# DIG-Beihang/RobustART

Hardware: AMD Instinct MI355X
Metric: corrupted+attacked images/sec/node (ResNet-50, PGD-7 + IN-C x5) (higher is better)
Workload: dtype bf16x3; 1 GPU; per step and GPU: gaussian_noise sev 1..5 on 256 u8 224x224 images -> normalise -> ResNet-50 eval (1280 img) + PGD-Linf-7 eps 2/255 ResNet-50 eval (256 img); global_batch=256, parallelism=dp1, streams=2

## Files before the change

### robustart_amd/csrc/stem_pair.hip

```cpp
#include "rart_common.h"

typedef __attribute__((ext_vector_type(8))) __bf16 bf16x8;
typedef __attribute__((ext_vector_type(4))) float f32x4;

namespace {
constexpr int T = 16;
constexpr int HT = T + 3;
constexpr int NPOS_PAD = 368;
constexpr int PT = T / 2 + 3;
constexpr int NPOOL = PT * PT;
constexpr int OT = 2 * T;
constexpr int OLD = OT + 1;
constexpr int DZ_BYTES = 2 * 4 * NPOS_PAD * 16;
constexpr int DP_BYTES = 2 * NPOOL * 4 * 16;
constexpr int ARG_BYTES = NPOOL * 4 * 8;
static_assert(3 * OT * OLD * 4 <= DP_BYTES + ARG_BYTES, "output tile must fit the raw pooled tile");

__device__ __forceinline__ uint32_t sp_pack2(float lo, float hi) {
  typedef __attribute__((ext_vector_type(2))) float f2;
  typedef __attribute__((ext_vector_type(2))) __bf16 b2;
  f2 f = {lo, hi};
  return __builtin_bit_cast(uint32_t, __builtin_convertvector(f, b2));
}

template <int EY, int EX>
__device__ __forceinline__ void pool_bwd_class_pair(uint4* sDz1, const uint4* sDp, const uint2* sArg, int tid, int a0, int b0, int qy0,
                                                    int qx0, int oh, int ow) {
  constexpr int NY = EY ? (HT + 1) / 2 : HT / 2, NX = EX ? (HT + 1) / 2 : HT / 2;
  constexpr int NYS = EY ? 2 : 1, NXS = EX ? 2 : 1;
  for (int i = tid; i < 4 * NY * NX; i += 256) {
    const int c = i / (NY * NX), j = i - c * (NY * NX);
    const int iy = j / NX, ix = j - iy * NX;
    const int hy = 2 * iy + (EY ? 0 : 1), hx = 2 * ix + (EX ? 0 : 1);
    const int py = a0 - 1 + hy, px = b0 - 1 + hx;
    float g[8] = {0.f, 0.f, 0.f, 0.f, 0.f, 0.f, 0.f, 0.f};
    if ((unsigned)py < (unsigned)oh && (unsigned)px < (unsigned)ow) {
#pragma unroll
      for (int ia = 0; ia < NYS; ++ia) {
        const int qy = (py >> 1) + ia;
        const uint32_t ky = (uint32_t)(py - (2 * qy - 1));
#pragma unroll
        for (int ib = 0; ib < NXS; ++ib) {
          const int qx = (px >> 1) + ib;
          const uint32_t mine = (ky * 3 + (uint32_t)(px - (2 * qx - 1))) * 0x01010101u;
          const int lp = (qy - qy0) * PT + (qx - qx0);
          const uint2 cd = sArg[c * NPOOL + lp];
          const uint4 dh = sDp[c * NPOOL + lp], dl = sDp[(4 + c) * NPOOL + lp];
          const uint32_t cw[2] = {cd.x, cd.y};
          const uint32_t hw_[4] = {dh.x, dh.y, dh.z, dh.w}, lw_[4] = {dl.x, dl.y, dl.z, dl.w};
#pragma unroll
          for (int hw = 0; hw < 2; ++hw) {
            const uint32_t ne = ((cw[hw] ^ mine) + 0x7F7F7F7Fu) & 0x80808080u;
            const uint32_t eq = (ne ^ 0x80808080u) >> 7;
            const uint32_t m = (eq << 8) - eq;
            const uint32_t m0 = __builtin_amdgcn_perm(m, m, 0x01010000u), m1 = __builtin_amdgcn_perm(m, m, 0x03030202u);
            const uint32_t h0 = hw_[2 * hw] & m0, h1 = hw_[2 * hw + 1] & m1, l0 = lw_[2 * hw] & m0, l1 = lw_[2 * hw + 1] & m1;
            g[4 * hw + 0] += __uint_as_float(h0 << 16) + __uint_as_float(l0 << 16);
            g[4 * hw + 1] += __uint_as_float(h0 & 0xFFFF0000u) + __uint_as_float(l0 & 0xFFFF0000u);
            g[4 * hw + 2] += __uint_as_float(h1 << 16) + __uint_as_float(l1 << 16);
            g[4 * hw + 3] += __uint_as_float(h1 & 0xFFFF0000u) + __uint_as_float(l1 & 0xFFFF0000u);
          }
        }
      }
    }
    uint32_t hv[4], lv[4];
#pragma unroll
    for (int k = 0; k < 4; ++k) {
      hv[k] = sp_pack2(g[2 * k], g[2 * k + 1]);
      lv[k] = sp_pack2(g[2 * k] - __uint_as_float(hv[k] << 16), g[2 * k + 1] - __uint_as_float(hv[k] & 0xFFFF0000u));
    }
    sDz1[c * NPOS_PAD + hy * HT + hx] = make_uint4(hv[0], hv[1], hv[2], hv[3]);
    sDz1[(4 + c) * NPOS_PAD + hy * HT + hx] = make_uint4(lv[0], lv[1], lv[2], lv[3]);
  }
}

struct Istd3p { float v[3]; };

__global__ __launch_bounds__(256, 2) void k_stem_bwd_pair(const uint4* __restrict__ dpool_h,
                                                          const uint4* __restrict__ dpool_l,
                                                          const uint4* __restrict__ arg,
                                                          const uint16_t* __restrict__ wt_h,
                                                          const uint16_t* __restrict__ wt_l,
                                                          float* __restrict__ grad,
                                                          int h, int w, Istd3p istd) {
  __shared__ __attribute__((aligned(16))) uint8_t lds[DZ_BYTES + DP_BYTES + ARG_BYTES];
  uint4* sDz1 = reinterpret_cast<uint4*>(lds);
  uint4* sDp = reinterpret_cast<uint4*>(lds + DZ_BYTES);
  uint2* sArg = reinterpret_cast<uint2*>(lds + DZ_BYTES + DP_BYTES);
  float* sOut = reinterpret_cast<float*>(lds + DZ_BYTES);

  const int tid = threadIdx.x, lane = tid & 63, wave = tid >> 6;
  const int oh = h >> 1, ow = w >> 1;
  const int oh2 = oh >> 1, ow2 = ow >> 1;
  const int a0 = blockIdx.y * T, b0 = blockIdx.x * T, img = blockIdx.z;
  const int qy0 = (a0 >> 1) - 1, qx0 = (b0 >> 1) - 1;
  const int fr = lane & 15, fg = lane >> 4;
  f32x4 acc[4];
#pragma unroll
  for (int m = 0; m < 4; ++m) acc[m] = (f32x4){0.f, 0.f, 0.f, 0.f};
  const uint4* wrow_h = reinterpret_cast<const uint4*>(wt_h + (size_t)fr * 1024 + fg * 8);
  const uint4* wrow_l = reinterpret_cast<const uint4*>(wt_l + (size_t)fr * 1024 + fg * 8);

#pragma unroll 1
  for (int half = 0; half < 2; ++half) {
    for (int i = tid; i < NPOOL * 10; i += 256) {
      const int pos = i / 10, v = i - pos * 10;
      const int qy = qy0 + pos / PT, qx = qx0 + pos % PT;
      const bool ok = (unsigned)qy < (unsigned)oh2 && (unsigned)qx < (unsigned)ow2;
      const size_t base = ((size_t)img * oh2 + qy) * ow2 + qx;
      if (v < 8) {
        const int pl = v >> 2, c = v & 3;
        uint4 val = make_uint4(0, 0, 0, 0);
        if (ok) val = (pl ? dpool_l : dpool_h)[base * 8 + half * 4 + c];
        sDp[(pl * 4 + c) * NPOOL + pos] = val;
      } else {
        uint4 val = make_uint4(0x0F0F0F0Fu, 0x0F0F0F0Fu, 0x0F0F0F0Fu, 0x0F0F0F0Fu);
        if (ok) val = arg[base * 4 + half * 2 + (v - 8)];
        sArg[(2 * (v - 8)) * NPOOL + pos] = make_uint2(val.x, val.y);
        sArg[(2 * (v - 8) + 1) * NPOOL + pos] = make_uint2(val.z, val.w);
      }
    }
    __syncthreads();
    pool_bwd_class_pair<0, 0>(sDz1, sDp, sArg, tid, a0, b0, qy0, qx0, oh, ow);
    pool_bwd_class_pair<0, 1>(sDz1, sDp, sArg, tid, a0, b0, qy0, qx0, oh, ow);
    pool_bwd_class_pair<1, 0>(sDz1, sDp, sArg, tid, a0, b0, qy0, qx0, oh, ow);
    pool_bwd_class_pair<1, 1>(sDz1, sDp, sArg, tid, a0, b0, qy0, qx0, oh, ow);
    __syncthreads();
#pragma unroll
    for (int dpi = 0; dpi < 4; ++dpi) {
      uint4 bh[4], bl[4];
#pragma unroll
      for (int t = 0; t < 4; ++t) {
        bh[t] = wrow_h[(dpi * 4 + t) * 8 + half * 4];
        bl[t] = wrow_l[(dpi * 4 + t) * 8 + half * 4];
      }
#pragma unroll
      for (int dqi = 0; dqi < 4; ++dqi) {
        const bf16x8 wh = __builtin_bit_cast(bf16x8, bh[dqi]), wl = __builtin_bit_cast(bf16x8, bl[dqi]);
#pragma unroll
        for (int m = 0; m < 4; ++m) {
          const int pos = (wave * 4 + m + dpi) * HT + fr + dqi;
          const bf16x8 ah = __builtin_bit_cast(bf16x8, sDz1[fg * NPOS_PAD + pos]);
          const bf16x8 al = __builtin_bit_cast(bf16x8, sDz1[(4 + fg) * NPOS_PAD + pos]);
          acc[m] = __builtin_amdgcn_mfma_f32_16x16x32_bf16(al, wh, acc[m], 0, 0, 0);
          acc[m] = __builtin_amdgcn_mfma_f32_16x16x32_bf16(ah, wl, acc[m], 0, 0, 0);
          acc[m] = __builtin_amdgcn_mfma_f32_16x16x32_bf16(ah, wh, acc[m], 0, 0, 0);
        }
      }
    }
  }

  if (fr < 12) {
    const int pq = fr / 3, c = fr - pq * 3;
    const int py = pq >> 1, px = pq & 1;
#pragma unroll
    for (int m = 0; m < 4; ++m)
#pragma unroll
      for (int j = 0; j < 4; ++j)
        sOut[(c * OT + 2 * (wave * 4 + m) + py) * OLD + 2 * (fg * 4 + j) + px] = acc[m][j];
  }
  __syncthreads();
  const size_t plane = (size_t)h * w;
  for (int i = tid; i < 3 * OT * (OT / 4); i += 256) {
    const int x4 = i & 7, row = i >> 3;
    const int c = row / OT, y = row - c * OT;
    const int gy = 2 * a0 + y, gx = 2 * b0 + x4 * 4;
    if (gy < h && gx < w) {
      const float s = istd.v[c];
      const float* r = sOut + (c * OT + y) * OLD + x4 * 4;
      *reinterpret_cast<float4*>(grad + ((size_t)img * 3 + c) * plane + (size_t)gy * w + gx) =
          make_float4(r[0] * s, r[1] * s, r[2] * s, r[3] * s);
    }
  }
}
}

extern "C" int rart_engine_stem_bwd_fused_pair(const void* dpool_hi, const void* dpool_lo, const void* argmax, const void* wtab_hi,
                                               const void* wtab_lo, float* grad, int n, int h, int w, const float* std_host,
                                               rart_stream_t stream) {
  RART_CHECK_ARG(dpool_hi && dpool_lo && argmax && wtab_hi && wtab_lo && grad && n > 0 && n <= 65535,
                 "rart_engine_stem_bwd_fused_pair: bad arguments");
  RART_CHECK_ARG(h % 4 == 0 && w % 4 == 0 && h >= 4 && w >= 4, "rart_engine_stem_bwd_fused_pair: h and w must be multiples of 4");
  Istd3p is;
  for (int c = 0; c < 3; ++c) is.v[c] = std_host ? 1.0f / std_host[c] : 1.0f;
  const int oh = h / 2, ow = w / 2;
  hipLaunchKernelGGL(k_stem_bwd_pair, dim3((ow + T - 1) / T, (oh + T - 1) / T, n), dim3(256), 0, (hipStream_t)stream,
                     (const uint4*)dpool_hi, (const uint4*)dpool_lo, (const uint4*)argmax, (const uint16_t*)wtab_hi,
                     (const uint16_t*)wtab_lo, grad, h, w, is);
  RART_CHECK_LAUNCH("rart_engine_stem_bwd_fused_pair");
  return RART_OK;
}

namespace {
typedef __attribute__((ext_vector_type(16))) float f32x16;
constexpr int SP_PT = 8;
constexpr int SP_R = 2 * SP_PT + 1;
constexpr int SP_NPOS = SP_R * SP_R;
constexpr int SP_PH = 2 * (SP_R - 1) + 7;
constexpr int SP_PW = 40;
constexpr int SP_PLANE = SP_PH * SP_PW * 8;
constexpr int SP_WROW = 464;
constexpr int SP_YROW = 272;
constexpr int SP_W_BYTES = 64 * SP_WROW;
constexpr int SP_T_BYTES = SP_NPOS * SP_YROW;
constexpr int SP_NT = 3;
static_assert(SP_T_BYTES >= 2 * SP_PLANE, "the stem-output tile must cover the patch it aliases");

struct StemNormP { float mean[3], istd[3]; };
#pragma clang fp contract(off)

template <bool SRC_U8>
__global__ __launch_bounds__(512, 1) void k_stem_fwd_pair(const void* __restrict__ src, const uint16_t* __restrict__ w_h,
                                                          const uint16_t* __restrict__ w_l, const float* __restrict__ bias,
                                                          uint4* __restrict__ p1_h, uint4* __restrict__ p1_l, uint2* __restrict__ arg,
                                                          uint8_t* __restrict__ sign, int n, int h, int w, StemNormP nm) {
  __shared__ __attribute__((aligned(16))) uint8_t lds[2 * SP_W_BYTES + SP_T_BYTES];
  uint8_t* sW = lds;
  uint8_t* sP = lds + 2 * SP_W_BYTES;
  const int tid = threadIdx.x, lane = tid & 63, wave = tid >> 6;
  const int wm = wave >> 1, wn = wave & 1;
  const int kq = lane >> 5;
  const int oh = h >> 1, ow = w >> 1, oh2 = oh >> 1, ow2 = ow >> 1;
  const int tiles_x = (ow2 + SP_PT - 1) / SP_PT, tiles_y = (oh2 + SP_PT - 1) / SP_PT;
  const int n_tiles = n * tiles_y * tiles_x;

  for (int i = tid; i < 2 * 64 * 28; i += 512) {
    const int pl = i / (64 * 28), j = i - pl * (64 * 28), row = j / 28, ch = j - row * 28;
    *reinterpret_cast<uint4*>(sW + pl * SP_W_BYTES + row * SP_WROW + ch * 16) =
        *reinterpret_cast<const uint4*>((pl ? w_l : w_h) + (size_t)row * 224 + ch * 8);
  }
  uint32_t a_off[SP_NT];
#pragma unroll
  for (int i = 0; i < SP_NT; ++i) {
    int p = (wm * SP_NT + i) * 32 + (lane & 31);
    p = p < SP_NPOS ? p : SP_NPOS - 1;
    const int py = p / SP_R, px = p - py * SP_R;
    a_off[i] = (uint32_t)(((2 * py) * SP_PW + 2 * px) * 8 + kq * 16);
  }
  const uint32_t w_off = (uint32_t)((wn * 32 + (lane & 31)) * SP_WROW + kq * 16);
  float bz[16];
#pragma unroll
  for (int r = 0; r < 16; ++r) bz[r] = bias ? bias[wn * 32 + (r & 3) + 8 * (r >> 2) + 4 * kq] : 0.f;

  for (int t = blockIdx.x; t < n_tiles; t += gridDim.x) {
    const int img = t / (tiles_y * tiles_x);
    const int tr = t - img * (tiles_y * tiles_x);
    const int q0y = (tr / tiles_x) * SP_PT, q0x = (tr % tiles_x) * SP_PT;
    const int in_y0 = 4 * q0y - 5, in_x0 = 4 * q0x - 5;
    __syncthreads();
    {
      constexpr int U = (SP_PH * SP_PW + 511) / 512;
      float v01[U][3];
      bool ok[U];
#pragma unroll
      for (int u = 0; u < U; ++u) {
        const int i = u * 512 + tid;
        const int pr = i / SP_PW, pc = i - pr * SP_PW;
        const int y = in_y0 + pr, x = in_x0 + pc;
        ok[u] = i < SP_PH * SP_PW && (unsigned)y < (unsigned)h && (unsigned)x < (unsigned)w && pc < SP_PH;
#pragma unroll
        for (int c = 0; c < 3; ++c) {
          v01[u][c] = 0.f;
          if (ok[u]) {
            if (SRC_U8) v01[u][c] = (float)((const uint8_t*)src)[(((size_t)img * h + y) * w + x) * 3 + c];
            else v01[u][c] = ((const float*)src)[(((size_t)img * 3 + c) * h + y) * w + x];
          }
        }
      }
#pragma unroll
      for (int u = 0; u < U; ++u) {
        const int i = u * 512 + tid;
        if (i >= SP_PH * SP_PW) continue;
        uint32_t hv[3] = {0, 0, 0}, lv[3] = {0, 0, 0};
        if (ok[u]) {
#pragma unroll
          for (int c = 0; c < 3; ++c) {
            const float x01 = SRC_U8 ? v01[u][c] * (1.0f / 255.0f) : v01[u][c];
            const float v = (x01 - nm.mean[c]) * nm.istd[c];
            hv[c] = sp_pack2(v, 0.f) & 0xFFFFu;
            lv[c] = sp_pack2(v - __uint_as_float(hv[c] << 16), 0.f) & 0xFFFFu;
          }
        }
        *reinterpret_cast<uint2*>(sP + i * 8) = make_uint2(hv[0] | (hv[1] << 16), hv[2]);
        *reinterpret_cast<uint2*>(sP + SP_PLANE + i * 8) = make_uint2(lv[0] | (lv[1] << 16), lv[2]);
      }
    }
    __syncthreads();
    f32x16 acc[SP_NT];
#pragma unroll
    for (int i = 0; i < SP_NT; ++i)
#pragma unroll
      for (int r = 0; r < 16; ++r) acc[i][r] = bz[r];
#pragma unroll
    for (int r = 0; r < 7; ++r)
#pragma unroll
      for (int ks = 0; ks < 2; ++ks) {
        const bf16x8 wh = *reinterpret_cast<const bf16x8*>(sW + w_off + r * 64 + ks * 32);
        const bf16x8 wl = *reinterpret_cast<const bf16x8*>(sW + SP_W_BYTES + w_off + r * 64 + ks * 32);
#pragma unroll
        for (int i = 0; i < SP_NT; ++i) {
          const bf16x8 ah = *reinterpret_cast<const bf16x8*>(sP + a_off[i] + r * (SP_PW * 8) + ks * 32);
          const bf16x8 al = *reinterpret_cast<const bf16x8*>(sP + a_off[i] + SP_PLANE + r * (SP_PW * 8) + ks * 32);
          acc[i] = __builtin_amdgcn_mfma_f32_32x32x16_bf16(wh, al, acc[i], 0, 0, 0);
          acc[i] = __builtin_amdgcn_mfma_f32_32x32x16_bf16(wl, ah, acc[i], 0, 0, 0);
          acc[i] = __builtin_amdgcn_mfma_f32_32x32x16_bf16(wh, ah, acc[i], 0, 0, 0);
        }
      }
    __syncthreads();
#pragma unroll
    for (int i = 0; i < SP_NT; ++i) {
      const int p = (wm * SP_NT + i) * 32 + (lane & 31);
      if (p < SP_NPOS) {
#pragma unroll
        for (int q = 0; q < 4; ++q) {
          float v[4];
#pragma unroll
          for (int k = 0; k < 4; ++k) v[k] = fmaxf(acc[i][4 * q + k], 0.f);
          const uint32_t h0 = sp_pack2(v[0], v[1]), h1 = sp_pack2(v[2], v[3]);
          const uint32_t l0 = sp_pack2(v[0] - __uint_as_float(h0 << 16), v[1] - __uint_as_float(h0 & 0xFFFF0000u));
          const uint32_t l1 = sp_pack2(v[2] - __uint_as_float(h1 << 16), v[3] - __uint_as_float(h1 & 0xFFFF0000u));
          *reinterpret_cast<float4*>(sP + p * SP_YROW + (wn * 32 + 8 * q + 4 * kq) * 4) =
              make_float4(__uint_as_float(h0 << 16) + __uint_as_float(l0 << 16), __uint_as_float(h0 & 0xFFFF0000u) + __uint_as_float(l0 & 0xFFFF0000u),
                          __uint_as_float(h1 << 16) + __uint_as_float(l1 << 16), __uint_as_float(h1 & 0xFFFF0000u) + __uint_as_float(l1 & 0xFFFF0000u));
        }
      }
    }
    __syncthreads();
    {
      const int c = tid & 7, q = tid >> 3;
      const int qy = q / SP_PT, qx = q - qy * SP_PT;
      const int gy = q0y + qy, gx = q0x + qx;
      if (gy < oh2 && gx < ow2) {
        float m[8];
        uint32_t code[8];
#pragma unroll
        for (int j = 0; j < 8; ++j) { m[j] = -INFINITY; code[j] = 0; }
        for (int ky = 0; ky < 3; ++ky) {
          const int y1 = 2 * gy - 1 + ky;
          if ((unsigned)y1 >= (unsigned)oh) continue;
          for (int kx = 0; kx < 3; ++kx) {
            const int x1 = 2 * gx - 1 + kx;
            if ((unsigned)x1 >= (unsigned)ow) continue;
            const float* tp = reinterpret_cast<const float*>(sP + ((2 * qy + ky) * SP_R + 2 * qx + kx) * SP_YROW) + c * 8;
            const float4 v0 = *reinterpret_cast<const float4*>(tp), v1 = *reinterpret_cast<const float4*>(tp + 4);
            const float f[8] = {v0.x, v0.y, v0.z, v0.w, v1.x, v1.y, v1.z, v1.w};
#pragma unroll
            for (int j = 0; j < 8; ++j)
              if (f[j] > m[j]) { m[j] = f[j]; code[j] = (uint32_t)(ky * 3 + kx); }
          }
        }
        const size_t o = (((size_t)img * oh2 + gy) * ow2 + gx) * 8 + c;
        uint32_t hv[4], lv[4];
#pragma unroll
        for (int k = 0; k < 4; ++k) {
          hv[k] = sp_pack2(m[2 * k], m[2 * k + 1]);
          lv[k] = sp_pack2(m[2 * k] - __uint_as_float(hv[k] << 16), m[2 * k + 1] - __uint_as_float(hv[k] & 0xFFFF0000u));
        }
        p1_h[o] = make_uint4(hv[0], hv[1], hv[2], hv[3]);
        p1_l[o] = make_uint4(lv[0], lv[1], lv[2], lv[3]);
        uint32_t sb = 0;
#pragma unroll
        for (int j = 0; j < 8; ++j) {
          if (m[j] > 0.f) sb |= 1u << j; else code[j] = 15u;
        }
        if (sign) sign[o] = (uint8_t)sb;
        if (arg) arg[o] = make_uint2(code[0] | (code[1] << 8) | (code[2] << 16) | (code[3] << 24),
                                     code[4] | (code[5] << 8) | (code[6] << 16) | (code[7] << 24));
      }
    }
  }
}
#pragma clang fp contract(fast)
}

extern "C" int rart_engine_stem_fwd_fused_pair(const void* src, int src_is_u8, const void* wgt_hi, const void* wgt_lo, const float* bias,
                                               void* p1_hi, void* p1_lo, void* argmax_out, void* sign_out, int n, int h, int w,
                                               const float* mean_host, const float* std_host, rart_stream_t stream) {
  RART_CHECK_ARG(src && wgt_hi && wgt_lo && p1_hi && p1_lo && n > 0 && h % 4 == 0 && w % 4 == 0 && h >= 4 && w >= 4,
                 "rart_engine_stem_fwd_fused_pair: bad arguments (h, w multiples of 4)");
  StemNormP nm;
  for (int c = 0; c < 3; ++c) {
    nm.mean[c] = mean_host ? mean_host[c] : 0.f;
    nm.istd[c] = std_host ? 1.0f / std_host[c] : 1.f;
  }
  const long long tiles = (long long)n * ((h / 4 + SP_PT - 1) / SP_PT) * ((w / 4 + SP_PT - 1) / SP_PT);
  const int grid = (int)(tiles < 256 ? tiles : 256);
  if (src_is_u8)
    hipLaunchKernelGGL(k_stem_fwd_pair<true>, dim3(grid), dim3(512), 0, (hipStream_t)stream, src, (const uint16_t*)wgt_hi,
                       (const uint16_t*)wgt_lo, bias, (uint4*)p1_hi, (uint4*)p1_lo, (uint2*)argmax_out, (uint8_t*)sign_out, n, h, w, nm);
  else
    hipLaunchKernelGGL(k_stem_fwd_pair<false>, dim3(grid), dim3(512), 0, (hipStream_t)stream, src, (const uint16_t*)wgt_hi,
                       (const uint16_t*)wgt_lo, bias, (uint4*)p1_hi, (uint4*)p1_lo, (uint2*)argmax_out, (uint8_t*)sign_out, n, h, w, nm);
  RART_CHECK_LAUNCH("rart_engine_stem_fwd_fused_pair");
  return RART_OK;
}
```

Measured before the change: 8228 images/s.

## Restructure stem kernels: prefetch next tiles, stage weights in LDS, pad layouts

In the stem backward kernel, the raw pooled-gradient and argmax tile for the next half is now loaded into registers while the current half is being computed. The MFMA weights are staged into LDS, in a region that aliases the raw tile, instead of being reloaded from global memory per pass. Pooled data moves to a padded, channel-interleaved layout to reduce LDS bank conflicts. The forward kernel prefetches the next tile's input patch (f32 path by default, u8 opt-in), pads the patch row stride, and rebalances m-tiles across waves. Optional timestamp instrumentation and profiling scripts are also added. The cost is more registers, more barriers, and a risk of lower occupancy.

```diff
diff --git a/profiles/stem_pair_ab.py b/profiles/stem_pair_ab.py
--- /dev/null
+++ b/profiles/stem_pair_ab.py
@@ -0,0 +1,73 @@
+import ctypes, json, os, subprocess, sys
+ROOT = os.path.dirname(os.path.dirname(os.path.abspath(__file__)))
+sys.path.insert(0, ROOT)
+
+if sys.argv[1] == '--kernels-child':
+    from robustart_amd import _lib
+    _lib.LIB_PATH = os.path.abspath(sys.argv[2])
+    import torch
+    from robustart_amd.model.engine import ResNet50Engine
+    from robustart_amd.model.engine_base import pair
+    lib = _lib.load()
+    B, H, W = 256, 224, 224
+    g = torch.Generator().manual_seed(5)
+    wb = torch.randn(64, 3, 7, 7, generator=g) * 0.1
+    wt = pair(ResNet50Engine._stem_bwd_table(wb, dtype=torch.float32)).cuda()
+    rows = torch.zeros(64, 7, 8, 4); rows[:, :, :7, :3] = wb.permute(0, 2, 3, 1)
+    wf = pair(rows.reshape(64, 224)).cuda()
+    bias = torch.randn(64, generator=g).cuda()
+    xf = torch.rand(B, 3, H, W, generator=g).cuda()
+    xu = torch.randint(0, 256, (B, H, W, 3), generator=g, dtype=torch.uint8).cuda()
+    p1 = torch.empty(2, B, H // 4, W // 4, 64, dtype=torch.bfloat16, device='cuda')
+    arg = torch.empty(B, H // 4, W // 4, 64, dtype=torch.uint8, device='cuda')
+    sign = torch.empty(B, H // 4, W // 4, 8, dtype=torch.uint8, device='cuda')
+    dp = pair(torch.randn(B, H // 4, W // 4, 64, generator=g)).cuda()
+    grad = torch.empty(B, 3, H, W, device='cuda')
+    m3 = (ctypes.c_float * 3)(0.485, 0.456, 0.406); s3 = (ctypes.c_float * 3)(0.229, 0.224, 0.225)
+    sp = _lib.stream_ptr()
+    fwd = lambda x, u8: _lib.check(lib.rart_engine_stem_fwd_fused_pair(_lib.ptr(x), u8, _lib.ptr(wf[0]), _lib.ptr(wf[1]), _lib.ptr(bias), _lib.ptr(p1[0]), _lib.ptr(p1[1]), _lib.ptr(arg), _lib.ptr(sign), B, H, W, m3, s3, sp))
+    bwd = lambda: _lib.check(lib.rart_engine_stem_bwd_fused_pair(_lib.ptr(dp[0]), _lib.ptr(dp[1]), _lib.ptr(arg), _lib.ptr(wt[0]), _lib.ptr(wt[1]), _lib.ptr(grad), B, H, W, s3, sp))
+    def t(fn, n=30):
+        for _ in range(5): fn()
+        torch.cuda.synchronize()
+        e0, e1 = torch.cuda.Event(enable_timing=True), torch.cuda.Event(enable_timing=True)
+        e0.record()
+        for _ in range(n): fn()
+        e1.record(); torch.cuda.synchronize()
+        return round(e0.elapsed_time(e1) / n * 1e3, 1)
+    print(json.dumps({'lib': sys.argv[2], 'fwd_f32_us': t(lambda: fwd(xf, 0)), 'fwd_u8_us': t(lambda: fwd(xu, 1)), 'bwd_us': t(bwd)}), flush=True)
+    sys.exit(0)
+if sys.argv[1] == '--bench-child':
+    import runpy
+    from robustart_amd import _lib
+    _lib.LIB_PATH = os.path.abspath(sys.argv[2])
+    sys.argv = [os.path.join(ROOT, 'bench.py')] + sys.argv[3:]
+    runpy.run_path(sys.argv[0], run_name='__main__')
+    sys.exit(0)
+
+mode, args = sys.argv[1], sys.argv[2:]
+rounds = int(args[args.index('--rounds') + 1]) if '--rounds' in args else (2 if mode == 'kernels' else 4)
+dump = args[args.index('--dump') + 1] if '--dump' in args else None
+libs = [a for a in args if a.endswith('.so')]
+for r in range(rounds):
+    for n, lib in enumerate(libs):
+        if mode == 'kernels':
+            cmd = [sys.executable, os.path.abspath(__file__), '--kernels-child', lib]
+        else:
+            cmd = [sys.executable, os.path.abspath(__file__), '--bench-child', lib, '--gpus', '1', '--steps', '20', '--warmup', '5']
+            if dump and r == 0:
+                cmd += ['--dump-outputs', os.path.join(dump, str(n))]
+        o = subprocess.run(cmd, capture_output=True, text=True, timeout=600)
+        line = [ln for ln in o.stdout.splitlines() if ln.startswith('{')]
+        if o.returncode != 0 or not line:
+            sys.exit('child failed for %s:\n%s' % (lib, o.stderr[-2000:]))
+        j = json.loads(line[-1])
+        print(json.dumps(j if mode == 'kernels' else {'lib': lib, 'round': r, 'ms_per_step': j['ms_per_step'], 'value': j['value']}), flush=True)
+if mode == 'bench' and dump:
+    import numpy as np
+    a, b = os.path.join(dump, '0'), os.path.join(dump, '1')
+    names = sorted(os.listdir(a))
+    assert names and names == sorted(os.listdir(b))
+    bad = [n for n in names if not np.array_equal(np.load(os.path.join(a, n)), np.load(os.path.join(b, n)))]
+    print(json.dumps({'dump_outputs_arrays': len(names), 'array_equal': not bad, 'different': bad}), flush=True)
+    sys.exit(1 if bad else 0)
diff --git a/profiles/stem_pair_lab_build.py b/profiles/stem_pair_lab_build.py
--- /dev/null
+++ b/profiles/stem_pair_lab_build.py
@@ -0,0 +1,23 @@
+import os
+import subprocess
+import sys
+
+ROOT = os.path.dirname(os.path.dirname(os.path.abspath(__file__)))
+sys.path.insert(0, ROOT)
+from robustart_amd.csrc import build as B
+
+
+def main(argv):
+    out, defs, src = argv[0], [a for a in argv[1:] if a.startswith('-D')], os.path.join(B.HERE, 'stem_pair.hip')
+    if '--source' in argv:
+        src = argv[argv.index('--source') + 1]
+    obj = out + '.stem_pair.o'
+    subprocess.check_call([B.HIPCC] + B.FLAGS + ['-I', B.HERE] + defs + ['-c', src, '-o', obj])
+    objs = [os.path.join(B.OBJ, f + '.o') for f in B.sources() if f != 'stem_pair.hip']
+    subprocess.check_call([B.HIPCC, '--offload-arch=gfx950', '-shared', '-fPIC', '-o', out] + objs + [obj])
+    os.remove(obj)
+    print('built', out)
+
+
+if __name__ == '__main__':
+    main(sys.argv[1:])
diff --git a/profiles/stem_pair_stamps.py b/profiles/stem_pair_stamps.py
--- /dev/null
+++ b/profiles/stem_pair_stamps.py
@@ -0,0 +1,44 @@
+import ctypes, json, os, sys
+ROOT = os.path.dirname(os.path.dirname(os.path.abspath(__file__)))
+sys.path.insert(0, ROOT)
+from robustart_amd import _lib
+_lib.LIB_PATH = os.path.abspath(sys.argv[1])
+import torch
+from robustart_amd.model.engine import ResNet50Engine
+from robustart_amd.model.engine_base import pair
+lib = _lib.load()
+B, H, W = 256, 224, 224
+g = torch.Generator().manual_seed(5)
+wb = torch.randn(64, 3, 7, 7, generator=g) * 0.1
+wt = pair(ResNet50Engine._stem_bwd_table(wb, dtype=torch.float32)).cuda()
+rows = torch.zeros(64, 7, 8, 4); rows[:, :, :7, :3] = wb.permute(0, 2, 3, 1)
+wf = pair(rows.reshape(64, 224)).cuda()
+bias = torch.randn(64, generator=g).cuda()
+xf = torch.rand(B, 3, H, W, generator=g).cuda()
+xu = torch.randint(0, 256, (B, H, W, 3), generator=g, dtype=torch.uint8).cuda()
+p1 = torch.empty(2, B, H // 4, W // 4, 64, dtype=torch.bfloat16, device='cuda')
+arg = torch.empty(B, H // 4, W // 4, 64, dtype=torch.uint8, device='cuda')
+sign = torch.empty(B, H // 4, W // 4, 8, dtype=torch.uint8, device='cuda')
+dp = pair(torch.randn(B, H // 4, W // 4, 64, generator=g)).cuda()
+grad = torch.empty(B, 3, H, W, device='cuda')
+m3 = (ctypes.c_float * 3)(0.485, 0.456, 0.406); s3 = (ctypes.c_float * 3)(0.229, 0.224, 0.225)
+sp = _lib.stream_ptr()
+fwd = lambda x, u8: _lib.check(lib.rart_engine_stem_fwd_fused_pair(_lib.ptr(x), u8, _lib.ptr(wf[0]), _lib.ptr(wf[1]), _lib.ptr(bias), _lib.ptr(p1[0]), _lib.ptr(p1[1]), _lib.ptr(arg), _lib.ptr(sign), B, H, W, m3, s3, sp))
+bwd = lambda: _lib.check(lib.rart_engine_stem_bwd_fused_pair(_lib.ptr(dp[0]), _lib.ptr(dp[1]), _lib.ptr(arg), _lib.ptr(wt[0]), _lib.ptr(wt[1]), _lib.ptr(grad), B, H, W, s3, sp))
+
+lib.rart_debug_stem_stamps.restype = ctypes.c_int
+lib.rart_debug_stem_stamps.argtypes = [ctypes.c_void_p, ctypes.c_int]
+buf = (ctypes.c_ulonglong * 16)()
+def stamps(fn, n=5):
+    for _ in range(3): fn()
+    torch.cuda.synchronize(); assert lib.rart_debug_stem_stamps(buf, 1) == 0
+    for _ in range(n): fn()
+    torch.cuda.synchronize(); assert lib.rart_debug_stem_stamps(buf, 1) == 0
+    return [int(v) for v in buf]
+out = {'lib': os.path.basename(sys.argv[1]), 'unit': 's_memtime ticks summed over waves; last entries = counts',
+       'fwd_names': ['stage(wait+convert+write)', 'mma(+next loads issue)', 'barrier after mma', 'relu+store tile', 'pool+global store', 'tiles*waves', 'whole loop', 'waves'],
+       'bwd_names': ['stage', 'pool backward', 'weights+mma', 'epilogue', 'whole kernel', 'waves']}
+v = stamps(lambda: fwd(xf, 0)); out['fwd_f32'] = v[8:16]
+v = stamps(lambda: fwd(xu, 1)); out['fwd_u8'] = v[8:16]
+v = stamps(bwd); out['bwd'] = v[0:6]
+print(json.dumps(out), flush=True)
diff --git a/robustart_amd/csrc/stem_pair.hip b/robustart_amd/csrc/stem_pair.hip
--- a/robustart_amd/csrc/stem_pair.hip
+++ b/robustart_amd/csrc/stem_pair.hip
@@ -1,20 +1,40 @@
 #include "rart_common.h"
+
+#include <type_traits>
 
 typedef __attribute__((ext_vector_type(8))) __bf16 bf16x8;
 typedef __attribute__((ext_vector_type(4))) float f32x4;
+
+#ifdef RART_STEM_STAMPS
+__device__ unsigned long long g_sp_stamps[2][8];
+#define SP_T(V) const unsigned long long V = __builtin_amdgcn_s_memtime();
+#define SP_ST(...) __VA_ARGS__
+#else
+#define SP_T(V)
+#define SP_ST(...)
+#endif
+#ifndef RART_STEM_U8_PREFETCH
+#define RART_STEM_U8_PREFETCH 0
+#endif
 
 namespace {
 constexpr int T = 16;
 constexpr int HT = T + 3;
 constexpr int NPOS_PAD = 368;
 constexpr int PT = T / 2 + 3;
+constexpr int PTS = 12;
 constexpr int NPOOL = PT * PT;
+constexpr int NPOOL_PAD = PT * PTS;
 constexpr int OT = 2 * T;
 constexpr int OLD = OT + 1;
+constexpr int OPL = OT * OLD + 3;
 constexpr int DZ_BYTES = 2 * 4 * NPOS_PAD * 16;
-constexpr int DP_BYTES = 2 * NPOOL * 4 * 16;
-constexpr int ARG_BYTES = NPOOL * 4 * 8;
-static_assert(3 * OT * OLD * 4 <= DP_BYTES + ARG_BYTES, "output tile must fit the raw pooled tile");
+constexpr int DP_BYTES = 2 * NPOOL_PAD * 4 * 16;
+constexpr int ARG_BYTES = NPOOL_PAD * 4 * 8;
+constexpr int W_BYTES = 2 * 16 * 64 * 16;
+constexpr int RW_BYTES = W_BYTES;
+static_assert(DP_BYTES + ARG_BYTES <= RW_BYTES && 3 * OPL * 4 <= RW_BYTES, "raw pooled tile and output tile must fit the weight region");
+static_assert(2 * (DZ_BYTES + RW_BYTES) <= 160 * 1024, "two workgroups per CU");
 
 __device__ __forceinline__ uint32_t sp_pack2(float lo, float hi) {
   typedef __attribute__((ext_vector_type(2))) float f2;
@@ -28,9 +48,10 @@
                                                     int qx0, int oh, int ow) {
   constexpr int NY = EY ? (HT + 1) / 2 : HT / 2, NX = EX ? (HT + 1) / 2 : HT / 2;
   constexpr int NYS = EY ? 2 : 1, NXS = EX ? 2 : 1;
-  for (int i = tid; i < 4 * NY * NX; i += 256) {
-    const int c = i / (NY * NX), j = i - c * (NY * NX);
-    const int iy = j / NX, ix = j - iy * NX;
+  for (int i = tid; i < ((4 * NY * PTS + 31) & ~31); i += 256) {
+    const int c = (i >> 3) & 3, j = (i & 7) + ((i >> 5) << 3);
+    const int iy = j / PTS, ix = j - iy * PTS;
+    if (iy >= NY || ix >= NX) continue;
     const int hy = 2 * iy + (EY ? 0 : 1), hx = 2 * ix + (EX ? 0 : 1);
     const int py = a0 - 1 + hy, px = b0 - 1 + hx;
     float g[8] = {0.f, 0.f, 0.f, 0.f, 0.f, 0.f, 0.f, 0.f};
@@ -43,9 +64,9 @@
         for (int ib = 0; ib < NXS; ++ib) {
           const int qx = (px >> 1) + ib;
           const uint32_t mine = (ky * 3 + (uint32_t)(px - (2 * qx - 1))) * 0x01010101u;
-          const int lp = (qy - qy0) * PT + (qx - qx0);
-          const uint2 cd = sArg[c * NPOOL + lp];
-          const uint4 dh = sDp[c * NPOOL + lp], dl = sDp[(4 + c) * NPOOL + lp];
+          const int lp = (qy - qy0) * PTS + (qx - qx0);
+          const uint2 cd = sArg[lp * 4 + c];
+          const uint4 dh = sDp[lp * 4 + c], dl = sDp[(NPOOL_PAD + lp) * 4 + c];
           const uint32_t cw[2] = {cd.x, cd.y};
           const uint32_t hw_[4] = {dh.x, dh.y, dh.z, dh.w}, lw_[4] = {dl.x, dl.y, dl.z, dl.w};
 #pragma unroll
@@ -83,10 +104,11 @@
                                                           const uint16_t* __restrict__ wt_l,
                                                           float* __restrict__ grad,
                                                           int h, int w, Istd3p istd) {
-  __shared__ __attribute__((aligned(16))) uint8_t lds[DZ_BYTES + DP_BYTES + ARG_BYTES];
+  __shared__ __attribute__((aligned(16))) uint8_t lds[DZ_BYTES + RW_BYTES];
   uint4* sDz1 = reinterpret_cast<uint4*>(lds);
   uint4* sDp = reinterpret_cast<uint4*>(lds + DZ_BYTES);
   uint2* sArg = reinterpret_cast<uint2*>(lds + DZ_BYTES + DP_BYTES);
+  uint4* sW = reinterpret_cast<uint4*>(lds + DZ_BYTES);
   float* sOut = reinterpret_cast<float*>(lds + DZ_BYTES);
 
   const int tid = threadIdx.x, lane = tid & 63, wave = tid >> 6;
@@ -98,45 +120,72 @@
   f32x4 acc[4];
 #pragma unroll
   for (int m = 0; m < 4; ++m) acc[m] = (f32x4){0.f, 0.f, 0.f, 0.f};
-  const uint4* wrow_h = reinterpret_cast<const uint4*>(wt_h + (size_t)fr * 1024 + fg * 8);
-  const uint4* wrow_l = reinterpret_cast<const uint4*>(wt_l + (size_t)fr * 1024 + fg * 8);
-
+  const uint4* wsrc_h = reinterpret_cast<const uint4*>(wt_h + (size_t)fr * 1024 + fg * 8) + wave * 8;
+  const uint4* wsrc_l = reinterpret_cast<const uint4*>(wt_l + (size_t)fr * 1024 + fg * 8) + wave * 8;
+
+  constexpr int SU = (NPOOL * 10 + 255) / 256;
+  uint4 sv[SU];
+  auto load_raw = [&](int half) {
+#pragma unroll
+    for (int u = 0; u < SU; ++u) {
+      const int i = u * 256 + tid;
+      const int pos = i / 10, v = i - pos * 10;
+      const int ry = pos / PT, rx = pos - ry * PT;
+      const int qy = qy0 + ry, qx = qx0 + rx;
+      const bool ok = i < NPOOL * 10 && (unsigned)qy < (unsigned)oh2 && (unsigned)qx < (unsigned)ow2;
+      const size_t base = ((size_t)img * oh2 + qy) * ow2 + qx;
+      sv[u] = v < 8 ? make_uint4(0, 0, 0, 0) : make_uint4(0x0F0F0F0Fu, 0x0F0F0F0Fu, 0x0F0F0F0Fu, 0x0F0F0F0Fu);
+      if (ok) sv[u] = v < 8 ? ((v >> 2) ? dpool_l : dpool_h)[base * 8 + half * 4 + (v & 3)] : arg[base * 4 + half * 2 + (v - 8)];
+    }
+  };
+  SP_ST(unsigned long long st[4] = {0, 0, 0, 0};)
+  SP_T(tb)
+  load_raw(0);
 #pragma unroll 1
   for (int half = 0; half < 2; ++half) {
-    for (int i = tid; i < NPOOL * 10; i += 256) {
+    SP_T(t0)
+#pragma unroll
+    for (int u = 0; u < SU; ++u) {
+      const int i = u * 256 + tid;
+      if (i >= NPOOL * 10) continue;
       const int pos = i / 10, v = i - pos * 10;
-      const int qy = qy0 + pos / PT, qx = qx0 + pos % PT;
-      const bool ok = (unsigned)qy < (unsigned)oh2 && (unsigned)qx < (unsigned)ow2;
-      const size_t base = ((size_t)img * oh2 + qy) * ow2 + qx;
+      const int ry = pos / PT, lp = ry * PTS + (pos - ry * PT);
       if (v < 8) {
-        const int pl = v >> 2, c = v & 3;
-        uint4 val = make_uint4(0, 0, 0, 0);
-        if (ok) val = (pl ? dpool_l : dpool_h)[base * 8 + half * 4 + c];
-        sDp[(pl * 4 + c) * NPOOL + pos] = val;
+        sDp[((v >> 2) * NPOOL_PAD + lp) * 4 + (v & 3)] = sv[u];
       } else {
-        uint4 val = make_uint4(0x0F0F0F0Fu, 0x0F0F0F0Fu, 0x0F0F0F0Fu, 0x0F0F0F0Fu);
-        if (ok) val = arg[base * 4 + half * 2 + (v - 8)];
-        sArg[(2 * (v - 8)) * NPOOL + pos] = make_uint2(val.x, val.y);
-        sArg[(2 * (v - 8) + 1) * NPOOL + pos] = make_uint2(val.z, val.w);
-      }
-    }
-    __syncthreads();
+        sArg[lp * 4 + 2 * (v - 8)] = make_uint2(sv[u].x, sv[u].y);
+        sArg[lp * 4 + 2 * (v - 8) + 1] = make_uint2(sv[u].z, sv[u].w);
+      }
+    }
+    __syncthreads();
+    SP_T(t1)
     pool_bwd_class_pair<0, 0>(sDz1, sDp, sArg, tid, a0, b0, qy0, qx0, oh, ow);
     pool_bwd_class_pair<0, 1>(sDz1, sDp, sArg, tid, a0, b0, qy0, qx0, oh, ow);
     pool_bwd_class_pair<1, 0>(sDz1, sDp, sArg, tid, a0, b0, qy0, qx0, oh, ow);
     pool_bwd_class_pair<1, 1>(sDz1, sDp, sArg, tid, a0, b0, qy0, qx0, oh, ow);
     __syncthreads();
+    SP_T(t2)
+    {
+      uint4 th[4], tl[4];
+#pragma unroll
+      for (int k = 0; k < 4; ++k) {
+        th[k] = wsrc_h[k * 32 + half * 4];
+        tl[k] = wsrc_l[k * 32 + half * 4];
+      }
+      if (half == 0) load_raw(1);
+#pragma unroll
+      for (int k = 0; k < 4; ++k) {
+        sW[(wave + 4 * k) * 64 + lane] = th[k];
+        sW[(16 + wave + 4 * k) * 64 + lane] = tl[k];
+      }
+    }
+    __syncthreads();
 #pragma unroll
     for (int dpi = 0; dpi < 4; ++dpi) {
-      uint4 bh[4], bl[4];
-#pragma unroll
-      for (int t = 0; t < 4; ++t) {
-        bh[t] = wrow_h[(dpi * 4 + t) * 8 + half * 4];
-        bl[t] = wrow_l[(dpi * 4 + t) * 8 + half * 4];
-      }
 #pragma unroll
       for (int dqi = 0; dqi < 4; ++dqi) {
-        const bf16x8 wh = __builtin_bit_cast(bf16x8, bh[dqi]), wl = __builtin_bit_cast(bf16x8, bl[dqi]);
+        const bf16x8 wh = __builtin_bit_cast(bf16x8, sW[(dpi * 4 + dqi) * 64 + lane]);
+        const bf16x8 wl = __builtin_bit_cast(bf16x8, sW[(16 + dpi * 4 + dqi) * 64 + lane]);
 #pragma unroll
         for (int m = 0; m < 4; ++m) {
           const int pos = (wave * 4 + m + dpi) * HT + fr + dqi;
@@ -148,8 +197,12 @@
         }
       }
     }
-  }
-
+    __syncthreads();
+    SP_T(t3)
+    SP_ST(st[0] += t1 - t0; st[1] += t2 - t1; st[2] += t3 - t2;)
+  }
+
+  SP_T(t4)
   if (fr < 12) {
     const int pq = fr / 3, c = fr - pq * 3;
     const int py = pq >> 1, px = pq & 1;
@@ -157,7 +210,7 @@
     for (int m = 0; m < 4; ++m)
 #pragma unroll
       for (int j = 0; j < 4; ++j)
-        sOut[(c * OT + 2 * (wave * 4 + m) + py) * OLD + 2 * (fg * 4 + j) + px] = acc[m][j];
+        sOut[c * OPL + (2 * (wave * 4 + m) + py) * OLD + 2 * (fg * 4 + j) + px] = acc[m][j];
   }
   __syncthreads();
   const size_t plane = (size_t)h * w;
@@ -167,11 +220,18 @@
     const int gy = 2 * a0 + y, gx = 2 * b0 + x4 * 4;
     if (gy < h && gx < w) {
       const float s = istd.v[c];
-      const float* r = sOut + (c * OT + y) * OLD + x4 * 4;
+      const float* r = sOut + c * OPL + y * OLD + x4 * 4;
       *reinterpret_cast<float4*>(grad + ((size_t)img * 3 + c) * plane + (size_t)gy * w + gx) =
           make_float4(r[0] * s, r[1] * s, r[2] * s, r[3] * s);
     }
   }
+  SP_T(t6)
+  SP_ST(if (lane == 0) {
+    for (int k = 0; k < 3; ++k) atomicAdd(&g_sp_stamps[0][k], st[k]);
+    atomicAdd(&g_sp_stamps[0][3], t6 - t4);
+    atomicAdd(&g_sp_stamps[0][4], t6 - tb);
+    atomicAdd(&g_sp_stamps[0][5], 1ull);
+  })
 }
 }
 
@@ -197,13 +257,18 @@
 constexpr int SP_R = 2 * SP_PT + 1;
 constexpr int SP_NPOS = SP_R * SP_R;
 constexpr int SP_PH = 2 * (SP_R - 1) + 7;
-constexpr int SP_PW = 40;
-constexpr int SP_PLANE = SP_PH * SP_PW * 8;
+constexpr int SP_SW = 40;
+constexpr int SP_PW = 49;
+constexpr int SP_ODD = 400;
+constexpr int SP_PLANE = (SP_PH + 1) / 2 * SP_PW * 16;
+__device__ __forceinline__ constexpr int sp_row_off(int row) { return (row >> 1) * (SP_PW * 16) + (row & 1) * SP_ODD; }
+static_assert(SP_ODD % 16 == 0 && SP_ODD >= SP_SW * 8 && SP_PW * 16 - SP_ODD >= SP_SW * 8, "both rows of a pair fit its stride");
 constexpr int SP_WROW = 464;
 constexpr int SP_YROW = 272;
 constexpr int SP_W_BYTES = 64 * SP_WROW;
 constexpr int SP_T_BYTES = SP_NPOS * SP_YROW;
 constexpr int SP_NT = 3;
+constexpr int SP_U = (SP_PH * SP_SW + 511) / 512;
 static_assert(SP_T_BYTES >= 2 * SP_PLANE, "the stem-output tile must cover the patch it aliases");
 
 struct StemNormP { float mean[3], istd[3]; };
@@ -229,88 +294,107 @@
     *reinterpret_cast<uint4*>(sW + pl * SP_W_BYTES + row * SP_WROW + ch * 16) =
         *reinterpret_cast<const uint4*>((pl ? w_l : w_h) + (size_t)row * 224 + ch * 8);
   }
+  const int mt0 = wm < 2 ? wm * SP_NT : 2 * SP_NT + (wm - 2) * (SP_NT - 1);
+  const int n_mt = wm < 2 ? SP_NT : SP_NT - 1;
   uint32_t a_off[SP_NT];
 #pragma unroll
   for (int i = 0; i < SP_NT; ++i) {
-    int p = (wm * SP_NT + i) * 32 + (lane & 31);
+    int p = (mt0 + i) * 32 + (lane & 31);
     p = p < SP_NPOS ? p : SP_NPOS - 1;
     const int py = p / SP_R, px = p - py * SP_R;
-    a_off[i] = (uint32_t)(((2 * py) * SP_PW + 2 * px) * 8 + kq * 16);
+    a_off[i] = (uint32_t)(py * (SP_PW * 16) + 2 * px * 8 + kq * 16);
   }
   const uint32_t w_off = (uint32_t)((wn * 32 + (lane & 31)) * SP_WROW + kq * 16);
   float bz[16];
 #pragma unroll
   for (int r = 0; r < 16; ++r) bz[r] = bias ? bias[wn * 32 + (r & 3) + 8 * (r >> 2) + 4 * kq] : 0.f;
 
+  constexpr bool PREFETCH = !SRC_U8 || RART_STEM_U8_PREFETCH;
+  float v01[SP_U][3];
+  bool ok[SP_U];
+  auto load_patch = [&](int t) {
+    const int img = t / (tiles_y * tiles_x);
+    const int tr = t - img * (tiles_y * tiles_x);
+    const int in_y0 = 4 * ((tr / tiles_x) * SP_PT) - 5, in_x0 = 4 * ((tr % tiles_x) * SP_PT) - 5;
+#pragma unroll
+    for (int u = 0; u < SP_U; ++u) {
+      const int i = u * 512 + tid;
+      const int pr = i / SP_SW, pc = i - pr * SP_SW;
+      const int y = in_y0 + pr, x = in_x0 + pc;
+      ok[u] = t < n_tiles && i < SP_PH * SP_SW && (unsigned)y < (unsigned)h && (unsigned)x < (unsigned)w && pc < SP_PH;
+#pragma unroll
+      for (int c = 0; c < 3; ++c) {
+        v01[u][c] = 0.f;
+        if (ok[u]) {
+          if (SRC_U8) v01[u][c] = (float)((const uint8_t*)src)[(((size_t)img * h + y) * w + x) * 3 + c];
+          else v01[u][c] = ((const float*)src)[(((size_t)img * 3 + c) * h + y) * w + x];
+        }
+      }
+    }
+  };
+  if (PREFETCH) load_patch(blockIdx.x);
+
+  SP_ST(unsigned long long fs[6] = {0, 0, 0, 0, 0, 0};)
+  SP_T(tf0)
   for (int t = blockIdx.x; t < n_tiles; t += gridDim.x) {
     const int img = t / (tiles_y * tiles_x);
     const int tr = t - img * (tiles_y * tiles_x);
     const int q0y = (tr / tiles_x) * SP_PT, q0x = (tr % tiles_x) * SP_PT;
-    const int in_y0 = 4 * q0y - 5, in_x0 = 4 * q0x - 5;
-    __syncthreads();
-    {
-      constexpr int U = (SP_PH * SP_PW + 511) / 512;
-      float v01[U][3];
-      bool ok[U];
-#pragma unroll
-      for (int u = 0; u < U; ++u) {
-        const int i = u * 512 + tid;
-        const int pr = i / SP_PW, pc = i - pr * SP_PW;
-        const int y = in_y0 + pr, x = in_x0 + pc;
-        ok[u] = i < SP_PH * SP_PW && (unsigned)y < (unsigned)h && (unsigned)x < (unsigned)w && pc < SP_PH;
+    if (!PREFETCH) load_patch(t);
+    SP_T(t0)
+    __syncthreads();
+#pragma unroll
+    for (int u = 0; u < SP_U; ++u) {
+      const int i = u * 512 + tid;
+      if (i >= SP_PH * SP_SW) continue;
+      const int pr = i / SP_SW, po = sp_row_off(pr) + (i - pr * SP_SW) * 8;
+      uint32_t hv[3] = {0, 0, 0}, lv[3] = {0, 0, 0};
+      if (ok[u]) {
 #pragma unroll
         for (int c = 0; c < 3; ++c) {
-          v01[u][c] = 0.f;
-          if (ok[u]) {
-            if (SRC_U8) v01[u][c] = (float)((const uint8_t*)src)[(((size_t)img * h + y) * w + x) * 3 + c];
-            else v01[u][c] = ((const float*)src)[(((size_t)img * 3 + c) * h + y) * w + x];
+          const float x01 = SRC_U8 ? v01[u][c] * (1.0f / 255.0f) : v01[u][c];
+          const float v = (x01 - nm.mean[c]) * nm.istd[c];
+          hv[c] = sp_pack2(v, 0.f) & 0xFFFFu;
+          lv[c] = sp_pack2(v - __uint_as_float(hv[c] << 16), 0.f) & 0xFFFFu;
+        }
+      }
+      *reinterpret_cast<uint2*>(sP + po) = make_uint2(hv[0] | (hv[1] << 16), hv[2]);
+      *reinterpret_cast<uint2*>(sP + SP_PLANE + po) = make_uint2(lv[0] | (lv[1] << 16), lv[2]);
+    }
+    __syncthreads();
+    SP_T(t1)
+    if (PREFETCH) load_patch(t + gridDim.x);
+    f32x16 acc[SP_NT];
+#pragma unroll
+    for (int i = 0; i < SP_NT; ++i)
+#pragma unroll
+      for (int r = 0; r < 16; ++r) acc[i][r] = bz[r];
+    auto row_taps = [&](auto nt) {
+#pragma unroll
+      for (int r = 0; r < 7; ++r)
+#pragma unroll
+        for (int ks = 0; ks < 2; ++ks) {
+          const bf16x8 wh = *reinterpret_cast<const bf16x8*>(sW + w_off + r * 64 + ks * 32);
+          const bf16x8 wl = *reinterpret_cast<const bf16x8*>(sW + SP_W_BYTES + w_off + r * 64 + ks * 32);
+#pragma unroll
+          for (int i = 0; i < decltype(nt)::value; ++i) {
+            const bf16x8 ah = *reinterpret_cast<const bf16x8*>(sP + a_off[i] + sp_row_off(r) + ks * 32);
+            const bf16x8 al = *reinterpret_cast<const bf16x8*>(sP + a_off[i] + SP_PLANE + sp_row_off(r) + ks * 32);
+            acc[i] = __builtin_amdgcn_mfma_f32_32x32x16_bf16(wh, al, acc[i], 0, 0, 0);
+            acc[i] = __builtin_amdgcn_mfma_f32_32x32x16_bf16(wl, ah, acc[i], 0, 0, 0);
+            acc[i] = __builtin_amdgcn_mfma_f32_32x32x16_bf16(wh, ah, acc[i], 0, 0, 0);
           }
         }
-      }
-#pragma unroll
-      for (int u = 0; u < U; ++u) {
-        const int i = u * 512 + tid;
-        if (i >= SP_PH * SP_PW) continue;
-        uint32_t hv[3] = {0, 0, 0}, lv[3] = {0, 0, 0};
-        if (ok[u]) {
-#pragma unroll
-          for (int c = 0; c < 3; ++c) {
-            const float x01 = SRC_U8 ? v01[u][c] * (1.0f / 255.0f) : v01[u][c];
-            const float v = (x01 - nm.mean[c]) * nm.istd[c];
-            hv[c] = sp_pack2(v, 0.f) & 0xFFFFu;
-            lv[c] = sp_pack2(v - __uint_as_float(hv[c] << 16), 0.f) & 0xFFFFu;
-          }
-        }
-        *reinterpret_cast<uint2*>(sP + i * 8) = make_uint2(hv[0] | (hv[1] << 16), hv[2]);
-        *reinterpret_cast<uint2*>(sP + SP_PLANE + i * 8) = make_uint2(lv[0] | (lv[1] << 16), lv[2]);
-      }
-    }
-    __syncthreads();
-    f32x16 acc[SP_NT];
-#pragma unroll
-    for (int i = 0; i < SP_NT; ++i)
-#pragma unroll
-      for (int r = 0; r < 16; ++r) acc[i][r] = bz[r];
-#pragma unroll
-    for (int r = 0; r < 7; ++r)
-#pragma unroll
-      for (int ks = 0; ks < 2; ++ks) {
-        const bf16x8 wh = *reinterpret_cast<const bf16x8*>(sW + w_off + r * 64 + ks * 32);
-        const bf16x8 wl = *reinterpret_cast<const bf16x8*>(sW + SP_W_BYTES + w_off + r * 64 + ks * 32);
-#pragma unroll
-        for (int i = 0; i < SP_NT; ++i) {
-          const bf16x8 ah = *reinterpret_cast<const bf16x8*>(sP + a_off[i] + r * (SP_PW * 8) + ks * 32);
-          const bf16x8 al = *reinterpret_cast<const bf16x8*>(sP + a_off[i] + SP_PLANE + r * (SP_PW * 8) + ks * 32);
-          acc[i] = __builtin_amdgcn_mfma_f32_32x32x16_bf16(wh, al, acc[i], 0, 0, 0);
-          acc[i] = __builtin_amdgcn_mfma_f32_32x32x16_bf16(wl, ah, acc[i], 0, 0, 0);
-          acc[i] = __builtin_amdgcn_mfma_f32_32x32x16_bf16(wh, ah, acc[i], 0, 0, 0);
-        }
-      }
-    __syncthreads();
+    };
+    if (wm < 2) row_taps(std::integral_constant<int, SP_NT>());
+    else row_taps(std::integral_constant<int, SP_NT - 1>());
+    SP_T(t2)
+    __syncthreads();
+    SP_T(t3)
 #pragma unroll
     for (int i = 0; i < SP_NT; ++i) {
-      const int p = (wm * SP_NT + i) * 32 + (lane & 31);
-      if (p < SP_NPOS) {
+      const int p = (mt0 + i) * 32 + (lane & 31);
+      if (i < n_mt && p < SP_NPOS) {
 #pragma unroll
         for (int q = 0; q < 4; ++q) {
           float v[4];
@@ -326,6 +410,7 @@
       }
     }
     __syncthreads();
+    SP_T(t4)
     {
       const int c = tid & 7, q = tid >> 3;
       const int qy = q / SP_PT, qx = q - qy * SP_PT;
@@ -368,7 +453,15 @@
                                      code[4] | (code[5] << 8) | (code[6] << 16) | (code[7] << 24));
       }
     }
-  }
+    SP_T(t5)
+    SP_ST(fs[0] += t1 - t0; fs[1] += t2 - t1; fs[2] += t3 - t2; fs[3] += t4 - t3; fs[4] += t5 - t4; fs[5] += 1;)
+  }
+  SP_T(tf1)
+  SP_ST(if (lane == 0) {
+    for (int k = 0; k < 6; ++k) atomicAdd(&g_sp_stamps[1][k], fs[k]);
+    atomicAdd(&g_sp_stamps[1][6], tf1 - tf0);
+    atomicAdd(&g_sp_stamps[1][7], 1ull);
+  })
 }
 #pragma clang fp contract(fast)
 }
@@ -394,3 +487,14 @@
   RART_CHECK_LAUNCH("rart_engine_stem_fwd_fused_pair");
   return RART_OK;
 }
+
+#ifdef RART_STEM_STAMPS
+extern "C" int rart_debug_stem_stamps(unsigned long long* out16, int reset) {
+  if (hipMemcpyFromSymbol(out16, HIP_SYMBOL(g_sp_stamps), sizeof(unsigned long long) * 16) != hipSuccess) return 1;
+  if (reset) {
+    unsigned long long z[16] = {0};
+    if (hipMemcpyToSymbol(HIP_SYMBOL(g_sp_stamps), z, sizeof(z)) != hipSuccess) return 1;
+  }
+  return 0;
+}
+#endif
```

After: 8337 images/s, median of 6. 1.01x the previous value.
